# bg5sbk/dragonboat

Hardware: AMD Instinct MI355X
Metric: quorum-commit decisions/sec (whole node) + % HBM roofline at 1/2/4/8 GPUs (higher is better)
Workload: dtype u64

## Files before the change

### dragonboat_amd/csrc/hq_wire.cpp

```cpp
#include <new>
#include <string>
#include <utility>
#include <vector>

#include "../../include/hipquorum.h"
#include "hq_stream.h"
#include "hq_wire_codec.h"
#include "hq_wire_dev.h"

namespace {

using hqw::kSnapshotReceived;

std::string message_error(const hqw::error &e) {
    switch (e.code) {
    case hqw::kVarintEnd: return "Message: unexpected end of data in a varint";
    case hqw::kVarintOverflow: return "Message: varint overflows 64 bits";
    case hqw::kFieldZero: return "Message: illegal field number 0";
    case hqw::kWrongType:
        return "Message: wrong wire type " + std::to_string(e.wt) + " for field " +
               std::to_string(e.field);
    case hqw::kGroup: return "Message: unsupported wire type (groups are not part of raft.proto)";
    case hqw::kFieldEnd: return "Message: unexpected end of data in a field";
    case hqw::kBytesEnd: return "Message: unexpected end of data in a length-delimited field";
// ... 154 lines not shown
    bool key(uint64_t id, uint32_t *k) {
        if (!worker) {
            *k = cluster(id);
            return true;
        }
        if (handle_of.find(id, k)) return true;
        uint32_t h;
        if (hq_worker_find(worker, id, &h) != HQ_OK) return false;
        bool fresh;
        handle_of.find_or_add(id, h, &fresh);
        *k = h;
        return true;
    }
    void resolve(size_t r0) {
        const size_t n = recs.size() - r0;
        size_t i = 0;
        for (; i < n; ++i) {
            if (worker && i + 8 < n) handle_of.prefetch(pending[i + 8]);
            if (!key(pending[i], &recs[r0 + i].key)) break;
        }
        if (i == n) return;
        size_t o = r0 + i;
        for (; i < n; ++i) {
            if (worker && i + 8 < n) handle_of.prefetch(pending[i + 8]);
            uint32_t k;
            if (!key(pending[i], &k)) {
                stats.dropped_no_cluster++;
                continue;
            }
            recs[o] = recs[r0 + i];
            recs[o++].key = k;
        }
        recs.resize(o);
    }
};

extern "C" {

int hq_wire_decode_batch(const uint8_t *bytes, size_t len, hq_wire_message *out, uint64_t cap,
                         uint64_t *count, hq_wire_batch_info *info) {
    if ((!bytes && len) || !count) return HQ_E_INVAL;
    hq_wire_batch_info bi;
    const int rc = hqw::walk_batch(
        bytes, len, bi,
        [&](size_t, size_t body, size_t n) {
            hq_wire_message tmp;
            hqw::error e;
            hq_wire_message &dst = out && bi.n_messages < cap ? out[bi.n_messages] : tmp;
            return hqw::decode_message(bytes + body, n, dst, e) ? HQ_OK : HQ_E_INVAL;
        },
        [] {});
    *count = bi.n_messages;
    if (rc) return rc;
    if (info) *info = bi;
    return *count > cap && out ? HQ_E_STATE : HQ_OK;
}

int hq_wire_encode_batch(const hq_wire_message *msgs, uint64_t n, uint64_t deployment_id,
                         const uint8_t *source, size_t source_len, uint8_t *out, uint64_t cap,
                         uint64_t *len) {
    if ((n && !msgs) || !len || (source_len && !source) || (cap && !out)) return HQ_E_INVAL;
    uint8_t *p = out, *const end = out + cap;
    for (uint64_t i = 0; i < n; ++i) {
        const hq_wire_message &m = msgs[i];
        if (m.n_entries) return HQ_E_INVAL;
        const uint64_t reject = m.ev.reject ? 1u : 0u;
        const uint64_t size = hqw::body_size(m.ev.type, m.to, m.ev.from, m.cluster_id, m.ev.term,
                                             m.log_term, m.ev.log_index, m.commit, reject, m.ev.hint,
                                             m.ev.hint_high);
        if ((uint64_t)(end - p) < size + 1 + hqw::vlen(size)) return HQ_E_STATE;
        p = hqw::put_field(p, 0x0a, size);
        p = hqw::put_body(p, m.ev.type, m.to, m.ev.from, m.cluster_id, m.ev.term, m.log_term,
                          m.ev.log_index, m.commit, reject, m.ev.hint, m.ev.hint_high);
    }
    if ((uint64_t)(end - p) < 1 + 10 + 1 + 10 + source_len + 1 + 10) return HQ_E_STATE;
    p = hqw::put_trailer(p, deployment_id, source, source_len);
    *len = (uint64_t)(p - out);
    return HQ_OK;
}

int hq_wire_open(uint64_t deployment_id, hq_wire **out) {
    if (!out) return HQ_E_INVAL;
    *out = new (std::nothrow) hq_wire();
    if (!*out) return HQ_E_NOMEM;
    (*out)->deployment_id = deployment_id;
    return HQ_OK;
}

void hq_wire_close(hq_wire *w) {
    if (w && w->dev) hq_wire_dev_close(w->dev);
    delete w;
}

const char *hq_wire_last_error(const hq_wire *w) { return w ? w->err.c_str() : ""; }

int hq_wire_attach(hq_wire *w, hq_worker *worker) {
    if (!w) return HQ_E_INVAL;
    if (!w->recs.empty() || w->dev_queued)
        return w->fail(HQ_E_STATE, "hq_wire_attach: events queued (reset first)");
    if (w->dev) {
        hq_wire_dev_close(w->dev);
        w->dev = nullptr;
        w->rejected = nullptr;
        w->n_rejected = 0;
    }
    w->worker = worker;
    w->handle_of = ClusterIndex();
    w->kcnt.clear();
    return HQ_OK;
}

int hq_wire_attach_device(hq_wire *w, hq_worker *worker) {
    if (!w) return HQ_E_INVAL;
    if (!worker) return w->fail(HQ_E_INVAL, "hq_wire_attach_device: NULL worker");
    if (!w->recs.empty() || w->dev_queued)
        return w->fail(HQ_E_STATE, "hq_wire_attach_device: events queued (reset first)");
    hq_wire_dev *dev = nullptr;
    const int rc = hq_wire_dev_open(worker, &dev);
    if (rc)
        return w->fail(rc, rc == HQ_E_INVAL ? "hq_wire_attach_device: not a device worker "
                                              "(HQ_WORKER_ON_DEVICE)"
                                            : "hq_wire_attach_device: device buffers");
    if (w->dev) hq_wire_dev_close(w->dev);
    w->dev = dev;
    w->rejected = nullptr;
    w->n_rejected = 0;
    w->worker = worker;
    w->handle_of = ClusterIndex();
    w->kcnt.clear();
    return HQ_OK;
}

int hq_wire_reset(hq_wire *w) {
    if (!w) return HQ_E_INVAL;
    if (w->dev) hq_wire_dev_reset(w->dev);
    w->batch_calls = 0;
    w->dev_queued = 0;
    w->rejected = nullptr;
    w->n_rejected = 0;
    w->recs.clear();
    std::fill(w->kcnt.begin(), w->kcnt.end(), 0u);
    w->clusters.clear();
    w->cluster_index.clear();
    w->stats = hq_wire_stats{};
    return HQ_OK;
}

int hq_wire_add_local(hq_wire *w, uint64_t cluster_id, const hq_event *events, uint64_t count) {
    if (!w || (count && !events)) return HQ_E_INVAL;
    const uint64_t off[2] = {0, count};
    return hq_wire_add_locals(w, 1, &cluster_id, off, events);
}

int hq_wire_add_locals(hq_wire *w, uint64_t n, const uint64_t *cluster_ids, const uint64_t *offsets,
                       const hq_event *events) {
    if (!w || (n && (!cluster_ids || !offsets))) return HQ_E_INVAL;
    if (n && offsets[n] > offsets[0] && !events) return HQ_E_INVAL;
    for (uint64_t c = 0; c < n; ++c) {
        if (offsets[c + 1] < offsets[c]) return w->fail(HQ_E_INVAL, "hq_wire_add_locals: offsets decrease");
        for (uint64_t i = offsets[c]; i < offsets[c + 1]; ++i) {
            switch (events[i].kind) {
            case HQ_EV_READ: case HQ_EV_CHECK_QUORUM: case HQ_EV_ELECTION: case HQ_EV_PROPOSE: break;
            default: return w->fail(HQ_E_INVAL, "hq_wire_add_local: kind must be a local event");
            }
        }
    }
    for (uint64_t c = 0; c < n; ++c) {
        if (offsets[c + 1] == offsets[c]) continue;
        uint32_t k;
        if (!w->key(cluster_ids[c], &k)) {
            w->stats.dropped_no_cluster += offsets[c + 1] - offsets[c];
            continue;
        }
        for (uint64_t i = offsets[c]; i < offsets[c + 1]; ++i) {
            const hq_event &e = events[i];
            Rec r{};
            r.key = k;
            r.cat = e.kind == HQ_EV_READ ? 0 : e.kind == HQ_EV_PROPOSE ? 3 : 2;
            r.kind = (uint8_t)e.kind;
            r.reject = e.reject != 0;
            r.type = e.type;
            r.from = e.from;
            r.term = e.term;
            r.log_index = e.log_index;
            r.hint = e.hint;
            r.hint_high = e.hint_high;
            w->recs.push_back(r);
            if (w->worker) w->count_key(k);
        }
    }
    return HQ_OK;
}

static int add_batch_device(hq_wire *w, const uint8_t *bytes, size_t len) {
    const uint32_t index = w->batch_calls++;
    if (hq_wire_dev_framing(w->dev)) {
        const int rc = hq_wire_dev_queue(w->dev, bytes, len, index);
        if (rc) return w->fail(rc, hq_wire_dev_error(w->dev));
        w->dev_queued++;
        return HQ_OK;
    }
    if (w->spans.empty()) w->spans.resize(1024);
    hq_wire_batch_info bi;
    uint64_t ns = 0;
    int rc = hq_wire_frame_batch(bytes, len, 0, w->spans.data(), w->spans.size(), &ns, &bi);
    if (rc == HQ_E_STATE) {
        w->spans.resize(ns);
        rc = hq_wire_frame_batch(bytes, len, 0, w->spans.data(), w->spans.size(), &ns, &bi);
    }
    if (rc) return w->fail(HQ_E_INVAL, "hq_wire_add_batch: malformed MessageBatch");
    w->stats.batches++;
    w->stats.bytes += len;
    if (bi.deployment_id != w->deployment_id || bi.bin_ver != HQ_RPC_BIN_VERSION) {
        w->stats.dropped_batches++;
        w->stats.dropped_messages += bi.n_messages;
        return HQ_OK;
    }
    if (bi.n_messages == 0) return HQ_OK;
    rc = hq_wire_dev_add_batch(w->dev, bytes, len, w->spans.data(), ns, bi.n_messages, index);
    if (rc) {
        w->stats.batches--;
        w->stats.bytes -= len;
        return w->fail(rc, hq_wire_dev_error(w->dev));
    }
    w->dev_queued += bi.n_messages;
    return HQ_OK;
}

int hq_wire_add_batch(hq_wire *w, const uint8_t *bytes, size_t len) {
    if (!w) return HQ_E_INVAL;
    if (!bytes && len) return w->fail(HQ_E_INVAL, "hq_wire_add_batch: NULL bytes");
    if (w->dev) return add_batch_device(w, bytes, len);
    const size_t r0 = w->recs.size();
    w->pending.clear();
    uint64_t entries = 0, snap = 0, no_cluster = 0;
    const bool now = w->worker != nullptr;
    constexpr size_t kAhead = 8;
    size_t looked = 0;
    auto look_up = [&]() {
        Rec &x = w->recs[r0 + looked];
        const uint64_t id = w->pending[looked++];
        if (w->handle_of.find(id, &x.key) || w->key(id, &x.key)) {
            w->count_key(x.key);
        } else {
            x.key = hq_wire::kNoKey;
            ++no_cluster;
        }
    };
    hqw::error err{};
    hq_wire_batch_info bi;
    auto on_message = [&](size_t, size_t body, size_t k) {
        const uint8_t *const m = bytes + body;
        Rec r;
        r.key = 0;
        r.pad = 0;
        r.pad2 = 0;
        uint64_t cid;
        uint32_t ent;
        if (!decode_marshal_order(m, k, r, cid, ent)) {
            hq_wire_message x;
            if (!hqw::decode_message(m, k, x, err)) return HQ_E_INVAL;
            r.kind = HQ_EV_MESSAGE;
            r.type = x.ev.type;
            r.from = x.ev.from;
            r.term = x.ev.term;
            r.log_index = x.ev.log_index;
            r.hint = x.ev.hint;
            r.hint_high = x.ev.hint_high;
            r.reject = x.ev.reject != 0;
            cid = x.cluster_id;
            ent = x.n_entries;
        }
        entries += ent;
        if (r.type == kSnapshotReceived) {
            ++snap;
            return HQ_OK;
        }
        r.cat = 1;
        w->recs.push_back(r);
        w->pending.push_back(cid);
        if (now) {
            w->handle_of.prefetch(cid);
            if (w->pending.size() - looked > kAhead) look_up();
        }
        return HQ_OK;
    };
    const int rc = hqw::walk_batch(bytes, len, bi, on_message, [] {});
    const uint64_t n = bi.n_messages;
    if (now) {
        while (looked < w->pending.size()) look_up();
        if (no_cluster && !rc) {
            size_t o = r0;
            for (size_t i = r0; i < w->recs.size(); ++i)
                if (w->recs[i].key != hq_wire::kNoKey) w->recs[o++] = w->recs[i];
            w->recs.resize(o);
        }
    }
    if (rc) {
        w->drop_from(r0);
        return w->fail(HQ_E_INVAL, "hq_wire_add_batch: malformed MessageBatch" +
                                       (err.code ? ": " + message_error(err) : std::string()));
    }
    w->stats.batches++;
    w->stats.bytes += len;
    if (bi.deployment_id != w->deployment_id || bi.bin_ver != HQ_RPC_BIN_VERSION) {
        w->drop_from(r0);
        w->stats.dropped_batches++;
        w->stats.dropped_messages += n;
        return HQ_OK;
    }
    w->stats.messages += n;
    w->stats.entries += entries;
    w->stats.snapshot_received += snap;
    w->stats.dropped_no_cluster += no_cluster;
    if (!now) w->resolve(r0);
    return HQ_OK;
}

int hq_wire_step_input(hq_wire *w, hq_worker *worker, hq_step_input *out, hq_wire_stats *stats) {
    if (!w || !worker || !out) return HQ_E_INVAL;
    if (w->worker) return w->fail(HQ_E_STATE, "hq_wire_step_input: attached (hq_wire_step_sized)");
    const uint32_t nc = (uint32_t)w->clusters.size();
    std::vector<uint32_t> handle(nc);
    std::vector<uint64_t> cnt((size_t)nc * 4 + 1, 0);
    for (uint32_t k = 0; k < nc; ++k)
        if (hq_worker_find(worker, w->clusters[k], &handle[k]) != HQ_OK) handle[k] = UINT32_MAX;
    for (const auto &r : w->recs) cnt[(size_t)r.key * 4 + r.cat + 1]++;
    for (size_t i = 1; i < cnt.size(); ++i) cnt[i] += cnt[i - 1];
    std::vector<uint32_t> perm(w->recs.size());
    std::vector<uint64_t> pos(cnt.begin(), cnt.end() - 1);
    for (uint32_t i = 0; i < (uint32_t)w->recs.size(); ++i) {
        const Rec &r = w->recs[i];
        perm[pos[(size_t)r.key * 4 + r.cat]++] = i;
    }
    w->groups.clear();
    w->offsets.assign(1, 0);
    w->events.clear();
    for (uint32_t k = 0; k < nc; ++k) {
        const uint64_t b = cnt[(size_t)k * 4], e = cnt[(size_t)k * 4 + 4];
        if (handle[k] == UINT32_MAX) {
            w->stats.dropped_no_cluster += e - b;
            continue;
        }
        if (b == e) continue;
        w->groups.push_back(handle[k]);
        for (uint64_t j = b; j < e; ++j) w->events.push_back(hqs::to_event(w->recs[perm[j]]));
        w->offsets.push_back(w->events.size());
    }
    out->n_groups = w->groups.size();
    out->groups = w->groups.data();
    out->offsets = w->offsets.data();
    out->events = w->events.data();
    if (stats) *stats = w->stats;
    return HQ_OK;
}

int hq_wire_step_stream(hq_wire *w, hq_worker *worker, hq_step_stream *out, hq_wire_stats *stats) {
    if (!w || !out) return HQ_E_INVAL;
    hq_step_input in;
    int rc = hq_wire_step_input(w, worker, &in, stats);
    if (rc) return rc;
    w->boffsets.resize(in.n_groups + 1);
    w->bytes.resize((size_t)w->events.size() * HQ_EVENT_STREAM_MAX);
    rc = hq_events_encode(in.n_groups, in.offsets, in.events, w->bytes.data(), w->bytes.size(),
                          w->boffsets.data());
    if (rc) return w->fail(rc, "hq_wire_step_stream: encode");
    out->n_groups = in.n_groups;
    out->groups = in.groups;
    out->offsets = in.offsets;
    out->boffsets = w->boffsets.data();
    out->bytes = w->bytes.data();
    out->sizes = nullptr;
    out->n_events = out->n_bytes = 0;
    out->sizes16 = nullptr;
    return HQ_OK;
}

int hq_wire_step_sized(hq_wire *w, uint8_t *bytes, uint64_t cap, uint16_t *sizes16, uint64_t n_cap,
                       hq_step_stream *out, hq_wire_stats *stats) {
    if (!w || !out || (cap && !bytes)) return HQ_E_INVAL;
    if (!w->worker) return w->fail(HQ_E_STATE, "hq_wire_step_sized: no worker attached");
    if (w->dev) return w->fail(HQ_E_STATE, "hq_wire_step_sized: device mode (hq_wire_step_device)");
    uint64_t n = 0;
    if (hq_worker_group_count(w->worker, &n) != HQ_OK) return HQ_E_INVAL;
    if (n > n_cap || (n && !sizes16))
        return w->fail(HQ_E_INVAL, "hq_wire_step_sized: sizes16 holds fewer words than the worker's groups");
    const uint32_t nr = (uint32_t)w->recs.size();
    w->cnt.assign(n + 1, 0);
    std::copy(w->kcnt.begin(), w->kcnt.begin() + std::min<size_t>(w->kcnt.size(), n + 1), w->cnt.begin());
    for (uint64_t h = 0; h < n; ++h) w->cnt[h + 1] += w->cnt[h];
    if (w->cnt[n] != nr) return w->fail(HQ_E_STATE, "hq_wire_step_sized: a queued record's handle is past the worker's groups");
    w->perm.resize(nr);
    w->pos.assign(w->cnt.begin(), w->cnt.end() - 1);
    for (uint32_t i = 0; i < nr; ++i) w->perm[w->pos[w->recs[i].key]++] = i;
    uint8_t *p = bytes, *const end = bytes + cap;
    uint64_t events = 0;
    for (uint64_t h = 0; h < n; ++h) {
        const uint32_t b = w->cnt[h], e = w->cnt[h + 1];
        uint8_t *const g0 = p;
        if (e > b) {
            w->grp.resize(e - b);
            Rec *g = w->grp.data();
            bool sorted = true;
            for (uint32_t j = b; j < e; ++j) {
                g[j - b] = w->recs[w->perm[j]];
                sorted = sorted && (j == b || g[j - b - 1].cat <= g[j - b].cat);
            }
            if (!sorted)
                for (uint32_t x = 1; x < e - b; ++x)
                    for (uint32_t y = x; y > 0 && g[y - 1].cat > g[y].cat; --y) std::swap(g[y - 1], g[y]);
            p = hqs::encode_group(p, end, static_cast<const hqs::WireEvent *>(g), e - b);
            if (!p) return w->fail(HQ_E_STATE, "hq_wire_step_sized: the stream does not fit cap");
            if (p - g0 > 0xFFFF || e - b > 0xFFFF)
                return w->fail(HQ_E_INVAL, "hq_wire_step_sized: a group of 2^16 events or bytes");
            events += e - b;
        }
        sizes16[h] = (uint16_t)(p - g0);
    }
    *out = hq_step_stream{};
    out->n_groups = n;
    out->bytes = bytes;
    out->sizes16 = sizes16;
    out->n_events = events;
    out->n_bytes = (uint64_t)(p - bytes);
    if (stats) *stats = w->stats;
    return HQ_OK;
}

int hq_wire_step_device(hq_wire *w, hq_step_output *out, hq_wire_stats *stats) {
    if (!w || !out) return HQ_E_INVAL;
    if (!w->dev) return w->fail(HQ_E_STATE, "hq_wire_step_device: no device worker attached");
    uint64_t c[4], rejected_bytes = 0, n_bad_message = 0;
    hq_wire_stats add{};
    const int rc = hq_wire_dev_step(w->dev, static_cast<const hqs::WireEvent *>(w->recs.data()),
                                    w->recs.size(), out, c, &w->rejected, &w->n_rejected,
                                    &rejected_bytes, &n_bad_message, &add);
    if (rc) return w->fail(rc, hq_wire_dev_error(w->dev));
    if (stats) {
        *stats = w->stats;
        stats->batches += add.batches;
        stats->bytes += add.bytes;
        stats->dropped_batches += add.dropped_batches;
        stats->dropped_messages += add.dropped_messages;
        stats->messages += c[0];
        stats->entries += c[1];
        stats->snapshot_received += c[2];
        stats->dropped_no_cluster += c[3];
        stats->batches -= n_bad_message;
        stats->bytes -= rejected_bytes;
    }
    return HQ_OK;
}

int hq_wire_set_device_framing(hq_wire *w, int on) {
    if (!w) return HQ_E_INVAL;
    if (!w->dev) return w->fail(HQ_E_STATE, "hq_wire_set_device_framing: no device worker attached");
    if (!w->recs.empty() || w->dev_queued)
        return w->fail(HQ_E_STATE, "hq_wire_set_device_framing: events queued (reset first)");
    hq_wire_dev_set_framing(w->dev, on != 0, w->deployment_id);
    return HQ_OK;
}

int hq_wire_device_frame_stats(hq_wire *w, uint64_t out[4]) {
    if (!w || !out) return HQ_E_INVAL;
    if (!w->dev) return w->fail(HQ_E_STATE, "hq_wire_device_frame_stats: no device worker attached");
    hq_wire_dev_frame_stats(w->dev, out);
    return HQ_OK;
}

int hq_wire_device_rejected(hq_wire *w, const uint32_t **batches, uint64_t *n) {
    if (!w || !batches || !n) return HQ_E_INVAL;
    if (!w->dev) return w->fail(HQ_E_STATE, "hq_wire_device_rejected: no device worker attached");
    *batches = w->rejected;
    *n = w->n_rejected;
    return HQ_OK;
}

}
```

### dragonboat_amd/csrc/hq_wire_dev.h

```cpp
#pragma once

#include <cstddef>
#include <cstdint>

#include "../../include/hipquorum.h"
#include "hq_stream.h"

struct hq_wire_dev;

int hq_wire_dev_open(hq_worker *worker, hq_wire_dev **out);
void hq_wire_dev_close(hq_wire_dev *d);
const char *hq_wire_dev_error(const hq_wire_dev *d);
void hq_wire_dev_reset(hq_wire_dev *d);
int hq_wire_dev_add_batch(hq_wire_dev *d, const uint8_t *bytes, size_t len, const hq_wire_span *spans,
                          uint64_t n_spans, uint64_t n_messages, uint32_t index);
void hq_wire_dev_set_framing(hq_wire_dev *d, bool on, uint64_t deployment_id);
bool hq_wire_dev_framing(const hq_wire_dev *d);
int hq_wire_dev_queue(hq_wire_dev *d, const uint8_t *bytes, size_t len, uint32_t index);
void hq_wire_dev_frame_stats(const hq_wire_dev *d, uint64_t out[4]);
int hq_wire_frame_launch(hq_ctx *ctx, const uint8_t *bytes, uint64_t len,
                         const hq_wire_batch_ref *batches, uint64_t n_batches, uint32_t segment_bytes,
                         uint64_t seg_cap, hq_wire_span *spans, uint64_t span_cap, uint32_t *span_batch,
                         hq_wire_frame_result *results, uint64_t *totals, uint32_t *voids,
                         const uint64_t *deployment_id);
int hq_wire_dev_step(hq_wire_dev *d, const hqs::WireEvent *locals, uint64_t n_locals,
                     hq_step_output *out, uint64_t counters[4], const uint32_t **rejected,
                     uint64_t *n_rejected, uint64_t *rejected_bytes, uint64_t *n_bad_message,
                     hq_wire_stats *add);
```

### dragonboat_amd/csrc/hq_wire_dev.hip

```cpp
#include <hipcub/hipcub.hpp>

#include <algorithm>
#include <cstring>
#include <new>

#include "hq_dstep.h"
#include "hq_internal.h"
#include "hq_wire_codec.h"
#include "hq_wire_dev.h"

namespace {

using hqw::kEmptyKey;
using hqw::kSnapshotReceived;
using hqw::Slot;

constexpr uint32_t kThreads = 256, kWaves = kThreads / 64;

struct WaveStage {
    uint4 bytes[(HQ_WIRE_SPAN_BYTES + 16) / 16];
    uint32_t pos[HQ_WIRE_SPAN_MESSAGES];
    uint32_t len[HQ_WIRE_SPAN_MESSAGES];
    uint32_t framed;
    uint32_t pad[3];
};

struct DecodeK {
    const uint8_t *bytes;
    uint64_t len;
    const hq_wire_span *spans;
    uint64_t n_spans;
    hq_wire_message *out;
    uint8_t *status;
    uint64_t n_messages;
    const uint32_t *span_batch;
    uint32_t *bad;
    hqs::WireEvent *recs;
    uint64_t *cids;
};

template <bool REC>
__global__ void __launch_bounds__(kThreads) k_wire_decode(const DecodeK a) {
    __shared__ WaveStage stage[kWaves];
    const uint32_t wave = threadIdx.x >> 6, lane = threadIdx.x & 63;
    const uint64_t s = (uint64_t)blockIdx.x * kWaves + wave;
    WaveStage &st = stage[wave];

    hq_wire_span sp{};
    if (s < a.n_spans) sp = a.spans[s];
    const bool large = (sp.flags & HQ_WIRE_SPAN_LARGE) != 0;
    const bool valid = sp.count >= 1 && sp.count <= HQ_WIRE_SPAN_MESSAGES && sp.offset <= a.len &&
                       sp.len <= a.len - sp.offset &&
                       (large ? sp.count == 1 : sp.len <= HQ_WIRE_SPAN_BYTES);
    const uint32_t count = sp.count <= HQ_WIRE_SPAN_MESSAGES ? sp.count : HQ_WIRE_SPAN_MESSAGES;
    const uint8_t *const g = a.bytes + sp.offset;
    const uint32_t L = (uint32_t)sp.len;
    const uint32_t sh = (uint32_t)(reinterpret_cast<uintptr_t>(g) & 15u);
    uint8_t *const sb = reinterpret_cast<uint8_t *>(st.bytes);

    if (valid && !large) {
        const uint4 *const g16 = reinterpret_cast<const uint4 *>(g - sh);
        const uint32_t words = (sh + L + 15) / 16;
        for (uint32_t c = lane; c < words; c += 64) {
            const uint32_t b0 = c * 16;
            if (b0 >= sh && b0 + 16 <= sh + L) {
                st.bytes[c] = g16[c];
            } else {
                for (uint32_t j = 0; j < 16; ++j)
                    if (b0 + j >= sh && b0 + j < sh + L) sb[b0 + j] = g[b0 + j - sh];
            }
        }
    }
    __syncthreads();

    if (valid && !large && lane == 0) {
        const uint8_t *const b = sb + sh;
        uint32_t p = 0, k = 0;
        for (; k < count; ++k) {
            uint64_t n;
            if (!hqw::header<uint32_t>(b, p, L, n)) break;
            st.pos[k] = p;
            st.len[k] = (uint32_t)n;
            p += (uint32_t)n;
        }
        st.framed = k == count && p == L;
    }
    __syncthreads();

    if (s >= a.n_spans || lane >= count) return;
    const uint64_t i = (uint64_t)sp.first + lane;
    if (i >= a.n_messages) return;
    bool ok = false;
    hq_wire_message m;
    hqw::error why;
    if (valid && !large) {
        if (st.framed) ok = hqw::decode_message<uint32_t>(sb + sh + st.pos[lane], st.len[lane], m, why);
    } else if (valid) {
        uint64_t p = 0, n;
        if (hqw::header<uint64_t>(g, p, sp.len, n) && p + n == sp.len)
            ok = hqw::decode_message<uint64_t>(g + p, n, m, why);
    }
    if (REC) {
        const uint32_t batch = a.span_batch[s];
        hqs::WireEvent r{};
        r.key = batch;
        r.cat = 1;
        r.kind = HQ_EV_MESSAGE;
        if (ok) {
            r.reject = m.ev.reject != 0;
            r.type = m.ev.type;
            r.pad2 = m.n_entries;
            r.from = m.ev.from;
            r.term = m.ev.term;
            r.log_index = m.ev.log_index;
            r.hint = m.ev.hint;
            r.hint_high = m.ev.hint_high;
            a.cids[i] = m.cluster_id;
        } else {
            a.bad[batch] = 1;
        }
        a.recs[i] = r;
    } else {
        if (ok) a.out[i] = m;
        a.status[i] = ok ? 0 : 1;
    }
}


struct KeysK {
    const hqs::WireEvent *recs;
    const uint64_t *cids;
    const uint32_t *bad;
    uint64_t n_msgs, n;
    const Slot *slots;
    uint64_t n_slots;
    uint32_t has_empty, empty_val;
    uint32_t sentinel;
    uint32_t *keys, *vals;
    unsigned long long *counters;
};

__device__ __forceinline__ unsigned long long wave_sum(unsigned long long v) {
    for (int d = 32; d; d >>= 1) v += __shfl_down(v, d, 64);
    return v;
}

__global__ void __launch_bounds__(256) k_wire_keys(const KeysK a) {
    const uint64_t i = (uint64_t)blockIdx.x * 256 + threadIdx.x;
    unsigned long long c[4] = {0, 0, 0, 0};
    if (i < a.n) {
        const hqs::WireEvent r = a.recs[i];
        uint32_t key = a.sentinel;
        if (i >= a.n_msgs) {
            key = r.key * 4 + r.cat;
        } else if (!a.bad[r.key]) {
            c[0] = 1;
            c[1] = r.pad2;
            if (r.type == kSnapshotReceived) {
                c[2] = 1;
            } else {
                uint32_t h = 0;
                if (hqw::find(a.slots, a.n_slots, a.has_empty, a.empty_val, a.cids[i], h)) key = h * 4 + 1;
                else c[3] = 1;
            }
        }
        a.keys[i] = key;
        a.vals[i] = (uint32_t)i;
    }
    for (int k = 0; k < 4; ++k) {
        const unsigned long long v = wave_sum(c[k]);
        if ((threadIdx.x & 63) == 0 && v) atomicAdd(&a.counters[k], v);
    }
}

__global__ void __launch_bounds__(256) k_wire_offsets(const uint32_t *keys, uint64_t n,
                                                      uint64_t n_groups, uint64_t *offsets) {
    const uint64_t h = (uint64_t)blockIdx.x * 256 + threadIdx.x;
    if (h > n_groups) return;
    const uint64_t want = h * 4;
    uint64_t lo = 0, hi = n;
    while (lo < hi) {
        const uint64_t mid = lo + (hi - lo) / 2;
        if (keys[mid] < want) lo = mid + 1;
        else hi = mid;
    }
    offsets[h] = lo;
}

__global__ void __launch_bounds__(256) k_wire_rows(const hqs::WireEvent *recs, const uint32_t *vals,
                                                   const uint64_t *n_rows, hq_event *events) {
    const uint64_t j = (uint64_t)blockIdx.x * 256 + threadIdx.x;
    if (j >= *n_rows) return;
    events[j] = hqs::to_event(recs[vals[j]]);
}

struct DevBuf {
    void *p = nullptr;
    size_t cap = 0;
};

struct StageBlock {
    uint8_t *host = nullptr, *dev = nullptr;
    size_t cap = 0, fill = 0;
};

}

extern "C" int hq_wire_decode_dev(hq_ctx *ctx, const uint8_t *bytes, uint64_t len,
                                  const hq_wire_span *spans, uint64_t n_spans, hq_wire_message *out,
                                  uint8_t *status, uint64_t n_messages) {
    if (!ctx) return HQ_E_INVAL;
    if (n_spans == 0 || n_messages == 0) return HQ_OK;
    if (!spans || !out || !status || (!bytes && len))
        return hq::fail(ctx, HQ_E_INVAL, "hq_wire_decode_dev: NULL argument");
    const uint64_t blocks = (n_spans + kWaves - 1) / kWaves;
    if (blocks > 0x7FFFFFFFull)
        return hq::fail(ctx, HQ_E_INVAL, "hq_wire_decode_dev: more than 2^33 spans");
    int rc = hq::pre_launch(ctx);
    if (rc) return rc;
    DecodeK k{};
    k.bytes = bytes;
    k.len = len;
    k.spans = spans;
    k.n_spans = n_spans;
    k.out = out;
    k.status = status;
    k.n_messages = n_messages;
    hipLaunchKernelGGL(k_wire_decode<false>, dim3((uint32_t)blocks), dim3(kThreads), 0, ctx->stream,
                       k);
    return hq::post_launch(ctx, "hq_wire_decode_dev");
}

struct hq_wire_dev {
    hq_worker *worker = nullptr;
    hq_ctx *ctx = nullptr;
    std::string err;
    std::vector<hq_wire_span> spans;
    std::vector<uint32_t> span_batch;
    std::vector<uint32_t> batch_index;
    std::vector<uint64_t> batch_len;
    uint64_t n_msgs = 0;
    std::vector<StageBlock> stage;
    std::vector<uint32_t> rejected;
    std::vector<Slot> slots;
    uint64_t known = 0;
    bool has_empty = false;
    uint32_t empty_val = 0;
    DevBuf d_slots, d_spans, d_span_batch, d_bad, d_recs, d_cids, d_keys, d_vals, d_events, d_offsets,
        d_counters, d_tmp;
    uint64_t *h_read = nullptr;
    uint32_t *h_bad = nullptr;
    size_t h_bad_cap = 0;
    bool framing = false;
    uint64_t deployment_id = 0;
    std::vector<hq_wire_batch_ref> refs;
    std::vector<const uint8_t *> host_bytes;
    std::vector<uint8_t> frame_rejected;
    DevBuf d_refs, d_frame;
    uint8_t *h_frame = nullptr;
    size_t h_frame_cap = 0;
    uint64_t frame_stats[4] = {0, 0, 0, 0};

    int fail(int code, const std::string &m) {
        err = m;
        return code;
    }
    int hip(hipError_t e, const char *what) {
        if (e == hipSuccess) return HQ_OK;
        return fail(e == hipErrorOutOfMemory ? HQ_E_NOMEM : HQ_E_DEVICE,
                    std::string(what) + ": " + hipGetErrorString(e));
    }
    int ensure(DevBuf &b, size_t bytes) {
        if (bytes <= b.cap) return HQ_OK;
        if (b.p) (void)hipFree(b.p);
        b.p = nullptr;
        b.cap = 0;
        const size_t want = std::max<size_t>(bytes + bytes / 2, 4096);
        const int rc = hip(hipMalloc(&b.p, want), "hq_wire device buffer");
        if (!rc) b.cap = want;
        return rc;
    }
    void insert(uint64_t id, uint32_t h) {
        uint32_t first;
        if (hqw::find(slots.data(), slots.size(), has_empty, empty_val, id, first)) return;
        if (id == kEmptyKey) {
            has_empty = true;
            empty_val = h;
            return;
        }
        const uint64_t mask = slots.size() - 1;
        uint64_t s = hqw::hash_id(id) & mask;
        while (slots[s].key != kEmptyKey) s = (s + 1) & mask;
        slots[s] = Slot{id, h, 0};
    }
    int extend(uint64_t G) {
        if (G == known && d_slots.p) return HQ_OK;
        size_t want = 1024;
        while (want < 2 * G) want *= 2;
        std::vector<uint64_t> ids(G);
        int rc = hq_worker_cluster_ids(worker, 0, G, ids.data());
        if (rc) return fail(rc, "hq_wire_step_device: the worker's groups");
        if (want != slots.size()) {
            slots.assign(want, Slot{kEmptyKey, 0, 0});
            has_empty = false;
            known = 0;
        }
        for (uint64_t h = known; h < G; ++h) insert(ids[h], (uint32_t)h);
        known = G;
        rc = ensure(d_slots, slots.size() * sizeof(Slot));
        if (!rc)
            rc = hip(hipMemcpyAsync(d_slots.p, slots.data(), slots.size() * sizeof(Slot),
                                    hipMemcpyHostToDevice, ctx->stream), "hq_wire table upload");
        return rc;
    }
};

int hq_wire_dev_open(hq_worker *worker, hq_wire_dev **out) {
    hq_ctx *ctx = hq_worker_device_ctx(worker);
    if (!ctx || !out) return HQ_E_INVAL;
    hq_wire_dev *d = new (std::nothrow) hq_wire_dev();
    if (!d) return HQ_E_NOMEM;
    d->worker = worker;
    d->ctx = ctx;
    int rc = d->hip(hipSetDevice(ctx->device), "hipSetDevice");
    if (!rc) rc = d->hip(hipHostMalloc(reinterpret_cast<void **>(&d->h_read), 64, hipHostMallocDefault),
                         "hq_wire pinned readback");
    if (rc) {
        delete d;
        return rc;
    }
    *out = d;
    return HQ_OK;
}

void hq_wire_dev_close(hq_wire_dev *d) {
    if (!d) return;
    (void)hipSetDevice(d->ctx->device);
    (void)hipStreamSynchronize(d->ctx->stream);
    for (DevBuf *b : {&d->d_slots, &d->d_spans, &d->d_span_batch, &d->d_bad, &d->d_recs, &d->d_cids,
                      &d->d_keys, &d->d_vals, &d->d_events, &d->d_offsets, &d->d_counters, &d->d_tmp,
                      &d->d_refs, &d->d_frame})
        if (b->p) (void)hipFree(b->p);
    for (StageBlock &s : d->stage)
        if (s.host) (void)hipHostFree(s.host);
    if (d->h_read) (void)hipHostFree(d->h_read);
    if (d->h_bad) (void)hipHostFree(d->h_bad);
    if (d->h_frame) (void)hipHostFree(d->h_frame);
    delete d;
}

const char *hq_wire_dev_error(const hq_wire_dev *d) { return d ? d->err.c_str() : ""; }

void hq_wire_dev_reset(hq_wire_dev *d) {
    d->spans.clear();
    d->span_batch.clear();
    d->batch_index.clear();
    d->batch_len.clear();
    d->n_msgs = 0;
    d->rejected.clear();
    d->refs.clear();
    d->host_bytes.clear();
    for (StageBlock &s : d->stage) s.fill = 0;
}

void hq_wire_dev_set_framing(hq_wire_dev *d, bool on, uint64_t deployment_id) {
    d->framing = on;
    d->deployment_id = deployment_id;
}

bool hq_wire_dev_framing(const hq_wire_dev *d) { return d->framing; }

void hq_wire_dev_frame_stats(const hq_wire_dev *d, uint64_t out[4]) {
    for (int k = 0; k < 4; ++k) out[k] = d->frame_stats[k];
}

static int place_batch(hq_wire_dev *d, const uint8_t *bytes, size_t len, const uint8_t **dev_out,
                       const uint8_t **host_out = nullptr) {
    int rc = d->hip(hipSetDevice(d->ctx->device), "hipSetDevice");
    if (rc) return rc;
    const uint8_t *dev = static_cast<const uint8_t *>(hq::device_view(bytes));
    if (host_out) *host_out = bytes;
    if (!dev) {
        StageBlock *blk = nullptr;
        for (StageBlock &s : d->stage)
            if (s.cap - s.fill >= len + 16) blk = &s;
        if (!blk) {
            StageBlock s;
            s.cap = std::max<size_t>(len + 16, size_t(4) << 20);
            rc = d->hip(hipHostMalloc(reinterpret_cast<void **>(&s.host), s.cap, hipHostMallocDefault),
                        "hq_wire pinned staging");
            if (!rc)
                rc = d->hip(hipHostGetDevicePointer(reinterpret_cast<void **>(&s.dev), s.host, 0),
                            "hq_wire pinned staging");
            if (rc) {
                if (s.host) (void)hipHostFree(s.host);
                return rc;
            }
            d->stage.push_back(s);
            blk = &d->stage.back();
        }
        std::memcpy(blk->host + blk->fill, bytes, len);
        dev = blk->dev + blk->fill;
        if (host_out) *host_out = blk->host + blk->fill;
        blk->fill += (len + 15) & ~size_t(15);
    }
    *dev_out = dev;
    return HQ_OK;
}

int hq_wire_dev_queue(hq_wire_dev *d, const uint8_t *bytes, size_t len, uint32_t index) {
    const uint8_t *dev = nullptr, *host = nullptr;
    if (len) {
        const int rc = place_batch(d, bytes, len, &dev, &host);
        if (rc) return rc;
    }
    d->batch_index.push_back(index);
    d->batch_len.push_back(len);
    d->refs.push_back(hq_wire_batch_ref{reinterpret_cast<uintptr_t>(dev), len});
    d->host_bytes.push_back(host);
    return HQ_OK;
}

int hq_wire_dev_add_batch(hq_wire_dev *d, const uint8_t *bytes, size_t len, const hq_wire_span *spans,
                          uint64_t n_spans, uint64_t n_messages, uint32_t index) {
    if (d->n_msgs + n_messages >= (1ull << 31))
        return d->fail(HQ_E_STATE, "hq_wire_add_batch: a device step holds < 2^31 messages");
    const uint8_t *dev = nullptr;
    const int rc = place_batch(d, bytes, len, &dev);
    if (rc) return rc;
    const uint32_t b = (uint32_t)d->batch_index.size();
    d->batch_index.push_back(index);
    d->batch_len.push_back(len);
    for (uint64_t i = 0; i < n_spans; ++i) {
        hq_wire_span s = spans[i];
        s.offset += reinterpret_cast<uintptr_t>(dev);
        s.first += (uint32_t)d->n_msgs;
        d->spans.push_back(s);
        d->span_batch.push_back(b);
    }
    d->n_msgs += n_messages;
    return HQ_OK;
}

static void queue_host_framed(hq_wire_dev *d, uint32_t b, const hq_wire_span *spans, uint64_t n_spans,
                              const hq_wire_batch_info &bi, hq_wire_stats *add) {
    add->batches++;
    add->bytes += d->batch_len[b];
    if (bi.deployment_id != d->deployment_id || bi.bin_ver != HQ_RPC_BIN_VERSION) {
        add->dropped_batches++;
        add->dropped_messages += bi.n_messages;
        return;
    }
    for (uint64_t i = 0; i < n_spans; ++i) {
        hq_wire_span s = spans[i];
        s.offset += d->refs[b].offset;
        s.first += (uint32_t)d->n_msgs;
        d->spans.push_back(s);
        d->span_batch.push_back(b);
    }
    d->n_msgs += bi.n_messages;
}

static int frame_queued(hq_wire_dev *d, hq_wire_stats *add, bool *on_device, uint64_t *n_spans) {
    hq_ctx *ctx = d->ctx;
    hipStream_t st = ctx->stream;
    const uint64_t nb = d->refs.size();
    const uint32_t S = HQ_WIRE_FRAME_SEGMENT, region = S / 128 + 8;
    uint64_t segs = 0;
    for (const hq_wire_batch_ref &r : d->refs) segs += (r.len + S - 1) / S;
    const uint64_t span_cap = segs * region;
    const size_t o_results = 16, o_voids = o_results + nb * sizeof(hq_wire_frame_result),
                 frame_bytes = o_voids + nb * 4;
    d->spans.clear();
    d->span_batch.clear();
    d->n_msgs = 0;
    d->frame_rejected.assign(nb, 0);
    d->frame_stats[0] = segs;
    d->frame_stats[1] = d->frame_stats[2] = 0;
    *on_device = false;
    *n_spans = 0;
    if (!nb) return HQ_OK;
    int rc = d->hip(hipSetDevice(ctx->device), "hipSetDevice");
    if (!rc) rc = d->ensure(d->d_refs, nb * sizeof(hq_wire_batch_ref));
    if (!rc) rc = d->ensure(d->d_frame, frame_bytes);
    if (!rc) rc = d->ensure(d->d_spans, span_cap * sizeof(hq_wire_span));
    if (!rc) rc = d->ensure(d->d_span_batch, span_cap * 4);
    if (!rc && frame_bytes > d->h_frame_cap) {
        if (d->h_frame) (void)hipHostFree(d->h_frame);
        d->h_frame = nullptr;
        d->h_frame_cap = 0;
        rc = d->hip(hipHostMalloc(reinterpret_cast<void **>(&d->h_frame), 2 * frame_bytes,
                                  hipHostMallocDefault), "hq_wire pinned readback");
        if (!rc) d->h_frame_cap = 2 * frame_bytes;
    }
    if (!rc)
        rc = d->hip(hipMemcpyAsync(d->d_refs.p, d->refs.data(), nb * sizeof(hq_wire_batch_ref),
                                   hipMemcpyHostToDevice, st), "hq_wire H2D");
    if (rc) return rc;
    uint8_t *const f = static_cast<uint8_t *>(d->d_frame.p);
    rc = hq_wire_frame_launch(ctx, nullptr, UINT64_MAX, static_cast<const hq_wire_batch_ref *>(d->d_refs.p),
                              nb, S, segs, static_cast<hq_wire_span *>(d->d_spans.p), span_cap,
                              static_cast<uint32_t *>(d->d_span_batch.p),
                              reinterpret_cast<hq_wire_frame_result *>(f + o_results),
                              reinterpret_cast<uint64_t *>(f), reinterpret_cast<uint32_t *>(f + o_voids),
                              &d->deployment_id);
    if (!rc) rc = hq::check_hip(ctx, hipMemcpyAsync(d->h_frame, f, frame_bytes, hipMemcpyDeviceToHost, st),
                                "hq_wire D2H");
    if (!rc) rc = hq::check_hip(ctx, hipStreamSynchronize(st), "hq_wire sync");
    if (rc) return d->fail(rc, ctx->err);
    const uint64_t *const totals = reinterpret_cast<const uint64_t *>(d->h_frame);
    const hq_wire_frame_result *const res =
        reinterpret_cast<const hq_wire_frame_result *>(d->h_frame + o_results);
    const uint32_t *const voids = reinterpret_cast<const uint32_t *>(d->h_frame + o_voids);
    for (uint64_t b = 0; b < nb; ++b) {
        d->frame_stats[1] += voids[b];
        d->frame_stats[2] += res[b].status >= 2;
    }
    if (d->frame_stats[2]) {
        d->frame_stats[3]++;
        std::vector<hq_wire_span> spans(1024);
        for (uint64_t b = 0; b < nb; ++b) {
            hq_wire_batch_info bi;
            uint64_t n = 0;
            int frc = hq_wire_frame_batch(d->host_bytes[b], d->batch_len[b], 0, spans.data(), spans.size(),
                                          &n, &bi);
            if (frc == HQ_E_STATE) {
                spans.resize(n);
                frc = hq_wire_frame_batch(d->host_bytes[b], d->batch_len[b], 0, spans.data(), spans.size(),
                                          &n, &bi);
            }
            if (frc) d->frame_rejected[b] = 1;
            else queue_host_framed(d, (uint32_t)b, spans.data(), n, bi, add);
        }
        *n_spans = d->spans.size();
        return HQ_OK;
    }
    for (uint64_t b = 0; b < nb; ++b) {
        if (res[b].status) {
            d->frame_rejected[b] = 1;
            continue;
        }
        hq_wire_batch_info bi{};
        bi.n_messages = res[b].n_messages;
        bi.deployment_id = res[b].deployment_id;
        bi.bin_ver = res[b].bin_ver;
        queue_host_framed(d, (uint32_t)b, nullptr, 0, bi, add);
    }
    if (d->n_msgs != totals[0])
        return d->fail(HQ_E_DEVICE, "hq_wire_step_device: the framing's totals differ from its results");
    *on_device = true;
    *n_spans = totals[1];
    return HQ_OK;
}

int hq_wire_dev_step(hq_wire_dev *d, const hqs::WireEvent *locals, uint64_t n_locals,
                     hq_step_output *out, uint64_t counters[4], const uint32_t **rejected,
                     uint64_t *n_rejected, uint64_t *rejected_bytes, uint64_t *n_bad_message,
                     hq_wire_stats *add) {
    hq_ctx *ctx = d->ctx;
    hipStream_t st = ctx->stream;
    std::memset(out, 0, sizeof *out);
    std::memset(counters, 0, 4 * sizeof(uint64_t));
    *add = hq_wire_stats{};
    d->rejected.clear();
    *rejected = nullptr;
    *n_rejected = *rejected_bytes = *n_bad_message = 0;
    int rc = HQ_OK;
    bool spans_on_device = false;
    uint64_t ns = d->spans.size();
    if (d->framing) {
        rc = frame_queued(d, add, &spans_on_device, &ns);
        if (rc) return rc;
        for (uint64_t b = 0; b < d->frame_rejected.size(); ++b)
            if (d->frame_rejected[b]) d->rejected.push_back(d->batch_index[b]);
        *rejected = d->rejected.data();
        *n_rejected = d->rejected.size();
    }
    const uint64_t nm = d->n_msgs, N = nm + n_locals, nb = d->batch_index.size();
    uint64_t G = 0;
    rc = hq_worker_group_count(d->worker, &G);
    if (rc) return d->fail(rc, "hq_wire_step_device: the worker's groups");
    if (N == 0 || G == 0) return HQ_OK;
    if (N >= (1ull << 31) || G >= (1ull << 30))
        return d->fail(HQ_E_STATE, "hq_wire_step_device: a step holds < 2^31 records, a worker < 2^30 groups");
    rc = d->hip(hipSetDevice(ctx->device), "hipSetDevice");
    if (!rc) rc = d->extend(G);
    size_t tmp = 0;
    const uint32_t sentinel = (uint32_t)(G * 4);
    int end_bit = 1;
    while (end_bit < 32 && (sentinel >> end_bit)) ++end_bit;
    if (!rc) rc = d->ensure(d->d_keys, 2 * N * 4);
    if (!rc) rc = d->ensure(d->d_vals, 2 * N * 4);
    uint32_t *keys_in = static_cast<uint32_t *>(d->d_keys.p), *keys_out = keys_in + N;
    uint32_t *vals_in = static_cast<uint32_t *>(d->d_vals.p), *vals_out = vals_in + N;
    if (!rc)
        rc = d->hip(hipcub::DeviceRadixSort::SortPairs(nullptr, tmp, keys_in, keys_out, vals_in,
                                                       vals_out, (int)N, 0, end_bit, st),
                    "hipcub sort size");
    if (!rc) rc = d->ensure(d->d_tmp, tmp);
    if (!rc && !spans_on_device) rc = d->ensure(d->d_spans, ns * sizeof(hq_wire_span));
    if (!rc && !spans_on_device) rc = d->ensure(d->d_span_batch, ns * 4);
    if (!rc) rc = d->ensure(d->d_bad, (nb + 1) * 4);
    if (!rc) rc = d->ensure(d->d_recs, N * sizeof(hqs::WireEvent));
    if (!rc) rc = d->ensure(d->d_cids, (nm + 1) * 8);
    if (!rc) rc = d->ensure(d->d_events, N * sizeof(hq_event));
    if (!rc) rc = d->ensure(d->d_offsets, (G + 1) * 8);
    if (!rc) rc = d->ensure(d->d_counters, 64);
    if (!rc && nb > d->h_bad_cap) {
        if (d->h_bad) (void)hipHostFree(d->h_bad);
        d->h_bad = nullptr;
        d->h_bad_cap = 0;
        rc = d->hip(hipHostMalloc(reinterpret_cast<void **>(&d->h_bad), nb * 2 * 4, hipHostMallocDefault),
                    "hq_wire pinned readback");
        if (!rc) d->h_bad_cap = nb * 2;
    }
    if (rc) return rc;
    hqs::WireEvent *recs = static_cast<hqs::WireEvent *>(d->d_recs.p);
    auto h2d = [&](void *dst, const void *src, size_t bytes) {
        if (!rc && bytes)
            rc = d->hip(hipMemcpyAsync(dst, src, bytes, hipMemcpyHostToDevice, st), "hq_wire H2D");
    };
    if (!spans_on_device) {
        h2d(d->d_spans.p, d->spans.data(), ns * sizeof(hq_wire_span));
        h2d(d->d_span_batch.p, d->span_batch.data(), ns * 4);
    }
    h2d(recs + nm, locals, n_locals * sizeof(hqs::WireEvent));
    if (!rc) rc = d->hip(hipMemsetAsync(d->d_bad.p, 0, (nb + 1) * 4, st), "memset");
    if (!rc) rc = d->hip(hipMemsetAsync(d->d_counters.p, 0, 64, st), "memset");
    if (rc) return rc;
    if (ns) {
        DecodeK k{};
        k.bytes = nullptr;
        k.len = UINT64_MAX;
        k.spans = static_cast<const hq_wire_span *>(d->d_spans.p);
        k.n_spans = ns;
        k.n_messages = nm;
        k.span_batch = static_cast<const uint32_t *>(d->d_span_batch.p);
        k.bad = static_cast<uint32_t *>(d->d_bad.p);
        k.recs = recs;
        k.cids = static_cast<uint64_t *>(d->d_cids.p);
        rc = hq::pre_launch(ctx);
        if (rc) return d->fail(rc, ctx->err);
        hipLaunchKernelGGL(k_wire_decode<true>, dim3((uint32_t)((ns + kWaves - 1) / kWaves)),
                           dim3(kThreads), 0, st, k);
        rc = hq::post_launch(ctx, "k_wire_decode");
        if (rc) return d->fail(rc, ctx->err);
    }
    KeysK kk{};
    kk.recs = recs;
    kk.cids = static_cast<const uint64_t *>(d->d_cids.p);
    kk.bad = static_cast<const uint32_t *>(d->d_bad.p);
    kk.n_msgs = nm;
    kk.n = N;
    kk.slots = static_cast<const Slot *>(d->d_slots.p);
    kk.n_slots = d->slots.size();
    kk.has_empty = d->has_empty;
    kk.empty_val = d->empty_val;
    kk.sentinel = sentinel;
    kk.keys = keys_in;
    kk.vals = vals_in;
    kk.counters = static_cast<unsigned long long *>(d->d_counters.p);
    uint64_t *offsets = static_cast<uint64_t *>(d->d_offsets.p);
    hq_event *events = static_cast<hq_event *>(d->d_events.p);
    rc = hq::pre_launch(ctx);
    if (rc) return d->fail(rc, ctx->err);
    hipLaunchKernelGGL(k_wire_keys, dim3((uint32_t)((N + 255) / 256)), dim3(256), 0, st, kk);
    rc = hq::post_launch(ctx, "k_wire_keys");
    if (!rc)
        rc = hq::check_hip(ctx, hipcub::DeviceRadixSort::SortPairs(d->d_tmp.p, tmp, keys_in, keys_out,
                                                                   vals_in, vals_out, (int)N, 0,
                                                                   end_bit, st), "hipcub sort");
    if (!rc) {
        hipLaunchKernelGGL(k_wire_offsets, dim3((uint32_t)((G + 1 + 255) / 256)), dim3(256), 0, st,
                           keys_out, N, G, offsets);
        rc = hq::post_launch(ctx, "k_wire_offsets");
    }
    if (!rc) {
        hipLaunchKernelGGL(k_wire_rows, dim3((uint32_t)((N + 255) / 256)), dim3(256), 0, st, recs,
                           vals_out, offsets + G, events);
        rc = hq::post_launch(ctx, "k_wire_rows");
    }
    if (!rc)
        rc = hq::check_hip(ctx, hipMemcpyAsync(d->h_read, d->d_counters.p, 32, hipMemcpyDeviceToHost, st),
                           "hq_wire D2H");
    if (!rc)
        rc = hq::check_hip(ctx, hipMemcpyAsync(d->h_read + 4, offsets + G, 8, hipMemcpyDeviceToHost, st),
                           "hq_wire D2H");
    if (!rc && nb)
        rc = hq::check_hip(ctx, hipMemcpyAsync(d->h_bad, d->d_bad.p, nb * 4, hipMemcpyDeviceToHost, st),
                           "hq_wire D2H");
    if (!rc) rc = hq::check_hip(ctx, hipStreamSynchronize(st), "hq_wire sync");
    if (rc) return d->fail(rc, ctx->err);
    for (int k = 0; k < 4; ++k) counters[k] = d->h_read[k];
    d->rejected.clear();
    for (uint64_t b = 0; b < nb; ++b) {
        if (d->framing && d->frame_rejected[b]) {
            d->rejected.push_back(d->batch_index[b]);
        } else if (d->h_bad[b]) {
            d->rejected.push_back(d->batch_index[b]);
            *rejected_bytes += d->batch_len[b];
            ++*n_bad_message;
        }
    }
    *rejected = d->rejected.data();
    *n_rejected = d->rejected.size();
    const uint64_t n_rows = d->h_read[4];
    if (n_rows == 0) return HQ_OK;
    rc = hq_worker_step_device_rows(d->worker, G, nullptr, offsets, events, n_rows, out);
    if (rc) return d->fail(rc, hq_worker_last_error(d->worker));
    return HQ_OK;
}
```

Measured before the change: 108.6 billion.

## Stage wire batches into HBM and resolve local-event cluster keys on device

Result: no change. 108.5 billion (-0.1%).

```diff
diff --git a/dragonboat_amd/csrc/hq_wire.cpp b/dragonboat_amd/csrc/hq_wire.cpp
--- a/dragonboat_amd/csrc/hq_wire.cpp
+++ b/dragonboat_amd/csrc/hq_wire.cpp
@@ -330,10 +330,50 @@
     return hq_wire_add_locals(w, 1, &cluster_id, off, events);
 }
 
+static int add_locals_device(hq_wire *w, uint64_t n, const uint64_t *cluster_ids,
+                             const uint64_t *offsets, const hq_event *events) {
+    for (uint64_t c = 0; c < n; ++c)
+        if (offsets[c + 1] < offsets[c]) return w->fail(HQ_E_INVAL, "hq_wire_add_locals: offsets decrease");
+    const uint64_t total = n ? offsets[n] - offsets[0] : 0;
+    if (!total) return HQ_OK;
+    Rec *recs = nullptr;
+    uint64_t *cids = nullptr;
+    const int rc = hq_wire_dev_reserve_locals(w->dev, total, &recs, &cids);
+    if (rc) return w->fail(rc, hq_wire_dev_error(w->dev));
+    uint64_t o = 0;
+    for (uint64_t c = 0; c < n; ++c) {
+        const uint64_t id = cluster_ids[c];
+        for (uint64_t i = offsets[c]; i < offsets[c + 1]; ++i, ++o) {
+            const hq_event &e = events[i];
+            Rec r{};
+            switch (e.kind) {
+            case HQ_EV_READ: r.cat = 0; break;
+            case HQ_EV_CHECK_QUORUM: case HQ_EV_ELECTION: r.cat = 2; break;
+            case HQ_EV_PROPOSE: r.cat = 3; break;
+            default: return w->fail(HQ_E_INVAL, "hq_wire_add_local: kind must be a local event");
+            }
+            r.kind = (uint8_t)e.kind;
+            r.reject = e.reject != 0;
+            r.type = e.type;
+            r.from = e.from;
+            r.term = e.term;
+            r.log_index = e.log_index;
+            r.hint = e.hint;
+            r.hint_high = e.hint_high;
+            recs[o] = r;
+            cids[o] = id;
+        }
+    }
+    hq_wire_dev_commit_locals(w->dev, total);
+    w->dev_queued += total;
+    return HQ_OK;
+}
+
 int hq_wire_add_locals(hq_wire *w, uint64_t n, const uint64_t *cluster_ids, const uint64_t *offsets,
                        const hq_event *events) {
     if (!w || (n && (!cluster_ids || !offsets))) return HQ_E_INVAL;
     if (n && offsets[n] > offsets[0] && !events) return HQ_E_INVAL;
+    if (w->dev) return add_locals_device(w, n, cluster_ids, offsets, events);
     for (uint64_t c = 0; c < n; ++c) {
         if (offsets[c + 1] < offsets[c]) return w->fail(HQ_E_INVAL, "hq_wire_add_locals: offsets decrease");
         for (uint64_t i = offsets[c]; i < offsets[c + 1]; ++i) {
@@ -610,9 +650,8 @@
     if (!w->dev) return w->fail(HQ_E_STATE, "hq_wire_step_device: no device worker attached");
     uint64_t c[4], rejected_bytes = 0, n_bad_message = 0;
     hq_wire_stats add{};
-    const int rc = hq_wire_dev_step(w->dev, static_cast<const hqs::WireEvent *>(w->recs.data()),
-                                    w->recs.size(), out, c, &w->rejected, &w->n_rejected,
-                                    &rejected_bytes, &n_bad_message, &add);
+    const int rc = hq_wire_dev_step(w->dev, out, c, &w->rejected, &w->n_rejected, &rejected_bytes,
+                                    &n_bad_message, &add);
     if (rc) return w->fail(rc, hq_wire_dev_error(w->dev));
     if (stats) {
         *stats = w->stats;
diff --git a/dragonboat_amd/csrc/hq_wire_dev.h b/dragonboat_amd/csrc/hq_wire_dev.h
--- a/dragonboat_amd/csrc/hq_wire_dev.h
+++ b/dragonboat_amd/csrc/hq_wire_dev.h
@@ -23,7 +23,8 @@
                          uint64_t seg_cap, hq_wire_span *spans, uint64_t span_cap, uint32_t *span_batch,
                          hq_wire_frame_result *results, uint64_t *totals, uint32_t *voids,
                          const uint64_t *deployment_id);
-int hq_wire_dev_step(hq_wire_dev *d, const hqs::WireEvent *locals, uint64_t n_locals,
-                     hq_step_output *out, uint64_t counters[4], const uint32_t **rejected,
-                     uint64_t *n_rejected, uint64_t *rejected_bytes, uint64_t *n_bad_message,
-                     hq_wire_stats *add);
+int hq_wire_dev_reserve_locals(hq_wire_dev *d, uint64_t n, hqs::WireEvent **recs, uint64_t **cids);
+void hq_wire_dev_commit_locals(hq_wire_dev *d, uint64_t n);
+int hq_wire_dev_step(hq_wire_dev *d, hq_step_output *out, uint64_t counters[4],
+                     const uint32_t **rejected, uint64_t *n_rejected, uint64_t *rejected_bytes,
+                     uint64_t *n_bad_message, hq_wire_stats *add);
diff --git a/dragonboat_amd/csrc/hq_wire_dev.hip b/dragonboat_amd/csrc/hq_wire_dev.hip
--- a/dragonboat_amd/csrc/hq_wire_dev.hip
+++ b/dragonboat_amd/csrc/hq_wire_dev.hip
@@ -152,7 +152,9 @@
         const hqs::WireEvent r = a.recs[i];
         uint32_t key = a.sentinel;
         if (i >= a.n_msgs) {
-            key = r.key * 4 + r.cat;
+            uint32_t h = 0;
+            if (hqw::find(a.slots, a.n_slots, a.has_empty, a.empty_val, a.cids[i], h)) key = h * 4 + r.cat;
+            else c[3] = 1;
         } else if (!a.bad[r.key]) {
             c[0] = 1;
             c[1] = r.pad2;
@@ -203,6 +205,20 @@
     uint8_t *host = nullptr, *dev = nullptr;
     size_t cap = 0, fill = 0;
 };
+
+struct DevBlock {
+    uint8_t *p = nullptr;
+    size_t cap = 0, fill = 0;
+};
+
+struct PendingCopy {
+    uint8_t *dst = nullptr;
+    const uint8_t *src = nullptr;
+    size_t len = 0, block = 0;
+    const uint8_t *owner = nullptr;
+};
+constexpr size_t kCopyAtOnce = size_t(4) << 20;
+constexpr size_t kDevBlockMin = size_t(256) << 10;
 
 }
 
@@ -241,6 +257,14 @@
     std::vector<uint64_t> batch_len;
     uint64_t n_msgs = 0;
     std::vector<StageBlock> stage;
+    std::vector<DevBlock> dev_stage;
+    size_t dev_cur = 0;
+    bool dev_stage_full = false;
+    PendingCopy pending;
+    bool copies_queued = false;
+    hqs::WireEvent *h_lrecs = nullptr;
+    uint64_t *h_lcids = nullptr;
+    uint64_t n_locals = 0, locals_cap = 0;
     std::vector<uint32_t> rejected;
     std::vector<Slot> slots;
     uint64_t known = 0;
@@ -343,6 +367,10 @@
         if (b->p) (void)hipFree(b->p);
     for (StageBlock &s : d->stage)
         if (s.host) (void)hipHostFree(s.host);
+    for (DevBlock &s : d->dev_stage)
+        if (s.p) (void)hipFree(s.p);
+    if (d->h_lrecs) (void)hipHostFree(d->h_lrecs);
+    if (d->h_lcids) (void)hipHostFree(d->h_lcids);
     if (d->h_read) (void)hipHostFree(d->h_read);
     if (d->h_bad) (void)hipHostFree(d->h_bad);
     if (d->h_frame) (void)hipHostFree(d->h_frame);
@@ -360,7 +388,17 @@
     d->rejected.clear();
     d->refs.clear();
     d->host_bytes.clear();
+    if (d->copies_queued) {
+        (void)hipSetDevice(d->ctx->device);
+        (void)hipStreamSynchronize(d->ctx->stream);
+        d->copies_queued = false;
+    }
+    d->pending.len = 0;
     for (StageBlock &s : d->stage) s.fill = 0;
+    for (DevBlock &s : d->dev_stage) s.fill = 0;
+    d->dev_cur = 0;
+    d->dev_stage_full = false;
+    d->n_locals = 0;
 }
 
 void hq_wire_dev_set_framing(hq_wire_dev *d, bool on, uint64_t deployment_id) {
@@ -372,13 +410,80 @@
 
 void hq_wire_dev_frame_stats(const hq_wire_dev *d, uint64_t out[4]) {
     for (int k = 0; k < 4; ++k) out[k] = d->frame_stats[k];
+}
+
+static int flush_copy(hq_wire_dev *d) {
+    PendingCopy &c = d->pending;
+    if (!c.len) return HQ_OK;
+    const size_t len = c.len;
+    c.len = 0;
+    d->copies_queued = true;
+    return d->hip(hipMemcpyAsync(c.dst, c.src, len, hipMemcpyHostToDevice, d->ctx->stream),
+                  "hq_wire batch copy");
+}
+
+static uint8_t *device_room(hq_wire_dev *d, const uint8_t *src, size_t len, size_t *block) {
+    const uintptr_t low = reinterpret_cast<uintptr_t>(src);
+    size_t total = 0;
+    for (size_t b = 0; b < d->dev_stage.size(); ++b) {
+        DevBlock &k = d->dev_stage[b];
+        total += k.cap;
+        if (b < d->dev_cur) continue;
+        const size_t at = k.fill + ((low - k.fill) & 15u);
+        if (at <= k.cap && len <= k.cap - at) {
+            d->dev_cur = b;
+            k.fill = at + len;
+            *block = b;
+            return k.p + at;
+        }
+    }
+    if (d->dev_stage_full) return nullptr;
+    DevBlock k;
+    k.cap = std::max(len + 16, std::max(kDevBlockMin, total));
+    if (hipMalloc(reinterpret_cast<void **>(&k.p), k.cap) != hipSuccess) {
+        (void)hipGetLastError();
+        d->dev_stage_full = true;
+        return nullptr;
+    }
+    const size_t at = low & 15u;
+    k.fill = at + len;
+    d->dev_stage.push_back(k);
+    d->dev_cur = *block = d->dev_stage.size() - 1;
+    return k.p + at;
+}
+
+static int copy_to_device(hq_wire_dev *d, const uint8_t *src, size_t len, const uint8_t *owner,
+                          const uint8_t **hbm) {
+    size_t block = 0;
+    uint8_t *const dst = device_room(d, src, len, &block);
+    *hbm = dst;
+    if (!dst) return HQ_OK;
+    PendingCopy &c = d->pending;
+    const uintptr_t s = reinterpret_cast<uintptr_t>(src), cs = reinterpret_cast<uintptr_t>(c.src);
+    const uintptr_t t = reinterpret_cast<uintptr_t>(dst), ct = reinterpret_cast<uintptr_t>(c.dst);
+    int rc = HQ_OK;
+    if (c.len && c.block == block && c.owner == owner && s >= cs + c.len &&
+        s - (cs + c.len) <= (owner ? 15u : 0u) && s - cs == t - ct) {
+        c.len = (s - cs) + len;
+    } else {
+        rc = flush_copy(d);
+        c.dst = dst;
+        c.src = src;
+        c.len = len;
+        c.block = block;
+        c.owner = owner;
+    }
+    if (!rc && c.len >= kCopyAtOnce) rc = flush_copy(d);
+    return rc;
 }
 
 static int place_batch(hq_wire_dev *d, const uint8_t *bytes, size_t len, const uint8_t **dev_out,
                        const uint8_t **host_out = nullptr) {
     int rc = d->hip(hipSetDevice(d->ctx->device), "hipSetDevice");
     if (rc) return rc;
-    const uint8_t *dev = static_cast<const uint8_t *>(hq::device_view(bytes));
+    bool pinned = false;
+    const uint8_t *dev = static_cast<const uint8_t *>(hq::device_view(bytes, &pinned));
+    const uint8_t *src = bytes, *owner = nullptr;
     if (host_out) *host_out = bytes;
     if (!dev) {
         StageBlock *blk = nullptr;
@@ -401,12 +506,58 @@
         }
         std::memcpy(blk->host + blk->fill, bytes, len);
         dev = blk->dev + blk->fill;
-        if (host_out) *host_out = blk->host + blk->fill;
+        src = blk->host + blk->fill;
+        owner = blk->host;
+        pinned = true;
+        if (host_out) *host_out = src;
         blk->fill += (len + 15) & ~size_t(15);
+    }
+    if (pinned && len) {
+        const uint8_t *hbm = nullptr;
+        rc = copy_to_device(d, src, len, owner, &hbm);
+        if (rc) return rc;
+        if (hbm) dev = hbm;
     }
     *dev_out = dev;
     return HQ_OK;
 }
+
+int hq_wire_dev_reserve_locals(hq_wire_dev *d, uint64_t n, hqs::WireEvent **recs, uint64_t **cids) {
+    int rc = d->hip(hipSetDevice(d->ctx->device), "hipSetDevice");
+    if (!rc) rc = flush_copy(d);
+    if (rc) return rc;
+    if (d->n_locals + n > d->locals_cap) {
+        const uint64_t cap = std::max<uint64_t>(std::max(2 * d->locals_cap, d->n_locals + n), 1024);
+        hqs::WireEvent *r = nullptr;
+        uint64_t *c = nullptr;
+        rc = d->hip(hipHostMalloc(reinterpret_cast<void **>(&r), cap * sizeof *r, hipHostMallocDefault),
+                    "hq_wire pinned local events");
+        if (!rc)
+            rc = d->hip(hipHostMalloc(reinterpret_cast<void **>(&c), cap * sizeof *c, hipHostMallocDefault),
+                        "hq_wire pinned local events");
+        if (!rc && d->copies_queued && d->h_lrecs)
+            rc = d->hip(hipStreamSynchronize(d->ctx->stream), "hq_wire sync");
+        if (rc) {
+            if (r) (void)hipHostFree(r);
+            if (c) (void)hipHostFree(c);
+            return rc;
+        }
+        if (d->n_locals) {
+            std::memcpy(r, d->h_lrecs, d->n_locals * sizeof *r);
+            std::memcpy(c, d->h_lcids, d->n_locals * sizeof *c);
+        }
+        if (d->h_lrecs) (void)hipHostFree(d->h_lrecs);
+        if (d->h_lcids) (void)hipHostFree(d->h_lcids);
+        d->h_lrecs = r;
+        d->h_lcids = c;
+        d->locals_cap = cap;
+    }
+    *recs = d->h_lrecs + d->n_locals;
+    *cids = d->h_lcids + d->n_locals;
+    return HQ_OK;
+}
+
+void hq_wire_dev_commit_locals(hq_wire_dev *d, uint64_t n) { d->n_locals += n; }
 
 int hq_wire_dev_queue(hq_wire_dev *d, const uint8_t *bytes, size_t len, uint32_t index) {
     const uint8_t *dev = nullptr, *host = nullptr;
@@ -553,19 +704,21 @@
     return HQ_OK;
 }
 
-int hq_wire_dev_step(hq_wire_dev *d, const hqs::WireEvent *locals, uint64_t n_locals,
-                     hq_step_output *out, uint64_t counters[4], const uint32_t **rejected,
-                     uint64_t *n_rejected, uint64_t *rejected_bytes, uint64_t *n_bad_message,
-                     hq_wire_stats *add) {
+int hq_wire_dev_step(hq_wire_dev *d, hq_step_output *out, uint64_t counters[4],
+                     const uint32_t **rejected, uint64_t *n_rejected, uint64_t *rejected_bytes,
+                     uint64_t *n_bad_message, hq_wire_stats *add) {
     hq_ctx *ctx = d->ctx;
     hipStream_t st = ctx->stream;
+    const uint64_t n_locals = d->n_locals;
     std::memset(out, 0, sizeof *out);
     std::memset(counters, 0, 4 * sizeof(uint64_t));
     *add = hq_wire_stats{};
     d->rejected.clear();
     *rejected = nullptr;
     *n_rejected = *rejected_bytes = *n_bad_message = 0;
-    int rc = HQ_OK;
+    int rc = d->hip(hipSetDevice(ctx->device), "hipSetDevice");
+    if (!rc) rc = flush_copy(d);
+    if (rc) return rc;
     bool spans_on_device = false;
     uint64_t ns = d->spans.size();
     if (d->framing) {
@@ -580,6 +733,7 @@
     uint64_t G = 0;
     rc = hq_worker_group_count(d->worker, &G);
     if (rc) return d->fail(rc, "hq_wire_step_device: the worker's groups");
+    if (G == 0) counters[3] = n_locals;
     if (N == 0 || G == 0) return HQ_OK;
     if (N >= (1ull << 31) || G >= (1ull << 30))
         return d->fail(HQ_E_STATE, "hq_wire_step_device: a step holds < 2^31 records, a worker < 2^30 groups");
@@ -602,7 +756,7 @@
     if (!rc && !spans_on_device) rc = d->ensure(d->d_span_batch, ns * 4);
     if (!rc) rc = d->ensure(d->d_bad, (nb + 1) * 4);
     if (!rc) rc = d->ensure(d->d_recs, N * sizeof(hqs::WireEvent));
-    if (!rc) rc = d->ensure(d->d_cids, (nm + 1) * 8);
+    if (!rc) rc = d->ensure(d->d_cids, (N + 1) * 8);
     if (!rc) rc = d->ensure(d->d_events, N * sizeof(hq_event));
     if (!rc) rc = d->ensure(d->d_offsets, (G + 1) * 8);
     if (!rc) rc = d->ensure(d->d_counters, 64);
@@ -624,7 +778,9 @@
         h2d(d->d_spans.p, d->spans.data(), ns * sizeof(hq_wire_span));
         h2d(d->d_span_batch.p, d->span_batch.data(), ns * 4);
     }
-    h2d(recs + nm, locals, n_locals * sizeof(hqs::WireEvent));
+    d->copies_queued = true;
+    h2d(recs + nm, d->h_lrecs, n_locals * sizeof(hqs::WireEvent));
+    h2d(static_cast<uint64_t *>(d->d_cids.p) + nm, d->h_lcids, n_locals * 8);
     if (!rc) rc = d->hip(hipMemsetAsync(d->d_bad.p, 0, (nb + 1) * 4, st), "memset");
     if (!rc) rc = d->hip(hipMemsetAsync(d->d_counters.p, 0, 64, st), "memset");
     if (rc) return rc;
@@ -691,6 +847,7 @@
                            "hq_wire D2H");
     if (!rc) rc = hq::check_hip(ctx, hipStreamSynchronize(st), "hq_wire sync");
     if (rc) return d->fail(rc, ctx->err);
+    d->copies_queued = false;
     for (int k = 0; k < 4; ++k) counters[k] = d->h_read[k];
     d->rejected.clear();
     for (uint64_t b = 0; b < nb; ++b) {
```
